# sulaimanvesal/PointCloudUDA

Hardware: AMD Instinct MI355X
Metric: adversarial train-step images/sec (seg+3 discr) at 256x256 (higher is better)
Workload: dtype bf16x3 MFMA (split-bf16, fp32 accumulate; fp32 storage); 1 GPU; MS-CMRSeg full UDA: UNet(PointNet head) + d1 + d2 + d4, 256x256x1, 4 classes; per_gpu_batch=32, global_batch=32, precision=bf16x3, parallelism=dp1, ranks_in_group=1, collective=none, streams=discriminators concurrent, d_target_forward=replayed from the adversarial pass of the same step, launch=eager (256 host cores for this rank)

## Files before the change

### pointcloududa_amd/csrc/conv_direct_d1.hip

```cpp
#include <stdlib.h>

#include "conv_host.h"
#include "conv_igemm.h"

namespace {

__device__ __forceinline__ float bf16_bits_to_float(uint16_t b) { return __builtin_bit_cast(float, (uint32_t)b << 16); }

bool direct_enabled(int bit) {
  static int mask = -1;
  if (mask < 0) {
    const char* e = getenv("PCUDA_NODIRECT");
    const char* m = getenv("PCUDA_DIRECT_MASK");
    mask = (e && atoi(e)) ? 0 : (m ? atoi(m) : 0x7f);
  }
  return (mask & bit) != 0;
}

struct D1Params {
  const float* dz; long long dz_sn, dz_sc;
  const float* x; long long x_sn, x_sc;
  float* dx; long long dx_sn, dx_sc;
  const uint16_t* wpack; int rec;
  float* partial;
  int accumulate;
  int n, h, w, oh, ow, cin, cout;
  long long cls_stride;
  int one;
};

template <int CIN>
__global__ __launch_bounds__(256) void d1_dgrad_kernel(const D1Params p) {
  __shared__ float sw[64 * CIN * 16];
  const int tid = threadIdx.x;
  for (int i = tid; i < p.cout * CIN * 16; i += 256) {
    const int kx = i & 3, ky = (i >> 2) & 3, ci = (i >> 4) % CIN, co = i / (16 * CIN);
    const int ry = ky & 1, rx = kx & 1, t = (ky >> 1) * 2 + (kx >> 1);
    const long long idx = (long long)(ry * 2 + rx) * p.cls_stride +
                          ((((long long)(co >> 5)) * 4 + t) * 32 + ci) * p.rec + (co & 31);
    const uint16_t* wq = p.wpack + idx;
    float v = bf16_bits_to_float(wq[0]);
    if (p.rec > IG_REC) v += bf16_bits_to_float(wq[32]);
    sw[i] = v;
    PCUDA_KEEP(wq);
  }
  __syncthreads();
  const int n = blockIdx.y;
  const int xg = p.w >> 3;
  const int item = blockIdx.x * 256 + tid;
  if (item >= xg * (p.h >> 1)) return;
  const int Y = item / xg, X0 = 4 * (item - Y * xg);
  float acc[CIN][2][8];
#pragma unroll
  for (int ci = 0; ci < CIN; ++ci)
#pragma unroll
    for (int r = 0; r < 2; ++r)
#pragma unroll
      for (int e = 0; e < 8; ++e) acc[ci][r][e] = 0.f;
  const float* zp = p.dz + (long long)n * p.dz_sn + (long long)Y * p.ow + X0;
  float zn[2][5];
  const float* zq[2];
#pragma unroll
  for (int a = 0; a < 2; ++a) {
    zq[a] = zp + a * p.ow;
#pragma unroll
    for (int b = 0; b < 5; ++b) zn[a][b] = zq[a][b * p.one];
  }
  for (int co = 0; co < p.cout; ++co) {
    float z[2][5];
    const float* zc[2];
#pragma unroll
    for (int a = 0; a < 2; ++a) {
      zc[a] = zq[a];
#pragma unroll
      for (int b = 0; b < 5; ++b) z[a][b] = zn[a][b];
    }
    const int con = min(co + 1, p.cout - 1);
#pragma unroll
    for (int a = 0; a < 2; ++a) {
      zq[a] = zp + (long long)con * p.dz_sc + a * p.ow;
#pragma unroll
      for (int b = 0; b < 5; ++b) zn[a][b] = zq[a][b * p.one];
    }
    const float* wc = sw + co * CIN * 16;
#pragma unroll
    for (int ci = 0; ci < CIN; ++ci)
#pragma unroll
      for (int py = 0; py < 2; ++py)
#pragma unroll
        for (int px = 0; px < 2; ++px)
#pragma unroll
          for (int a = 0; a < 2; ++a)
#pragma unroll
            for (int b = 0; b < 2; ++b) {
              const float wv = wc[(ci * 4 + py + 2 * (1 - a)) * 4 + px + 2 * (1 - b)];
#pragma unroll
              for (int j = 0; j < 4; ++j) acc[ci][py][2 * j + px] = fmaf(wv, z[a][j + b], acc[ci][py][2 * j + px]);
            }
    PCUDA_KEEP(zc[0]); PCUDA_KEEP(zc[1]);
  }
  PCUDA_KEEP(zq[0]); PCUDA_KEEP(zq[1]);
#pragma unroll
  for (int ci = 0; ci < CIN; ++ci)
#pragma unroll
    for (int r = 0; r < 2; ++r) {
      float* d = p.dx + (long long)n * p.dx_sn + (long long)ci * p.dx_sc + (long long)(2 * Y + r) * p.w + 2 * X0;
      f32x4 o0 = {acc[ci][r][0], acc[ci][r][1], acc[ci][r][2], acc[ci][r][3]};
      f32x4 o1 = {acc[ci][r][4], acc[ci][r][5], acc[ci][r][6], acc[ci][r][7]};
      if (p.accumulate) {
        const f32x4 q0 = *(const f32x4*)d, q1 = *(const f32x4*)(d + 4);
#pragma unroll
        for (int e = 0; e < 4; ++e) { o0[e] += q0[e]; o1[e] += q1[e]; }
      }
      *(f32x4*)d = o0;
      *(f32x4*)(d + 4) = o1;
    }
}

#define D1_ZP 132
#define D1_XP 276
template <int CIN>
__global__ __launch_bounds__(256) void d1_wgrad_kernel(const D1Params p, const int items) {
  extern __shared__ __attribute__((aligned(16))) float smem_f[];
  float* sz = smem_f;
  float* sx = smem_f + 64 * D1_ZP;
  const int tid = threadIdx.x;
  const int cg = tid >> 4, jg = tid & 15;
  const int ci = jg >> 2, ky = jg & 3;
  const bool live = ci < CIN;
  float acc[4][4];
#pragma unroll
  for (int c = 0; c < 4; ++c)
#pragma unroll
    for (int k = 0; k < 4; ++k) acc[c][k] = 0.f;
  const int ow4 = (p.ow + 3) >> 2;
  const int lane = tid & 63, wv = __builtin_amdgcn_readfirstlane(tid >> 6);
  float rz[16][3];
  f32x4 rx[4];
  const float* xq[4] = {p.x, p.x, p.x, p.x};
  const unsigned zoff[3] = {(unsigned)min(lane, p.ow - 1), (unsigned)min(lane + 64, p.ow - 1), (unsigned)min(lane + 128, p.ow - 1)};
  const unsigned xoff = (unsigned)min(4 * lane, p.w - 4);
  auto issue = [&](int it) {
    const int n = it / p.oh, oy = it - n * p.oh;
    const float* zb = p.dz + (long long)n * p.dz_sn + (long long)oy * p.ow;
#pragma unroll
    for (int k = 0; k < 16; ++k) {
      const float* zrow = zb + (long long)min(wv + 4 * k, p.cout - 1) * p.dz_sc;
#pragma unroll
      for (int u = 0; u < 3; ++u) rz[k][u] = zrow[zoff[u]];
    }
    const float* xb = p.x + (long long)n * p.x_sn + (long long)min(wv, CIN - 1) * p.x_sc;
#pragma unroll
    for (int r = 0; r < 4; ++r) {
      const float* xrow = xb + (long long)min(max(2 * oy + r - 2, 0), p.h - 1) * p.w;
      xq[r] = xrow + xoff;
      rx[r] = *(const f32x4*)xq[r];
    }
  };
  auto commit = [&](int it) {
    const int n = it / p.oh, oy = it - n * p.oh;
    (void)n;
#pragma unroll
    for (int k = 0; k < 16; ++k) {
      const int co = wv + 4 * k;
#pragma unroll
      for (int u = 0; u < 3; ++u) {
        const int c = lane + 64 * u;
        if (c < D1_ZP) sz[co * D1_ZP + c] = (c < p.ow && co < p.cout) ? rz[k][u] : 0.f;
      }
    }
    if (wv < CIN) {
#pragma unroll
      for (int r = 0; r < 4; ++r) {
        const int yy = 2 * oy + r - 2;
        const bool ok = (unsigned)yy < (unsigned)p.h && 4 * lane < p.w;
        float* d = sx + (wv * 4 + r) * D1_XP + 2 + 4 * lane;
#pragma unroll
        for (int e = 0; e < 4; ++e) d[e] = ok ? rx[r][e] : 0.f;
        PCUDA_KEEP(xq[r]);
        if (lane < 2) sx[(wv * 4 + r) * D1_XP + lane] = 0.f;
        if (lane < D1_XP - 2 - 256) sx[(wv * 4 + r) * D1_XP + 2 + 256 + lane] = 0.f;
      }
    }
  };
  int it = blockIdx.x;
  if (it < items) issue(it);
  for (; it < items; it += gridDim.x) {
    __syncthreads();
    commit(it);
    __syncthreads();
    const int nit = it + gridDim.x;
    if (nit < items) issue(nit);
    if (live) {
      const float* xr = sx + (ci * 4 + ky) * D1_XP;
      for (int q = 0; q < ow4; ++q) {
        const f32x4 x0 = *(const f32x4*)(xr + 8 * q), x1 = *(const f32x4*)(xr + 8 * q + 4), x2 = *(const f32x4*)(xr + 8 * q + 8);
        const float xv[12] = {x0[0], x0[1], x0[2], x0[3], x1[0], x1[1], x1[2], x1[3], x2[0], x2[1], x2[2], x2[3]};
#pragma unroll
        for (int c = 0; c < 4; ++c) {
          const f32x4 z = *(const f32x4*)(sz + (cg * 4 + c) * D1_ZP + 4 * q);
#pragma unroll
          for (int j = 0; j < 4; ++j)
#pragma unroll
            for (int kx = 0; kx < 4; ++kx) acc[c][kx] = fmaf(z[j], xv[2 * j + kx], acc[c][kx]);
        }
      }
    }
  }
  PCUDA_KEEP(zoff[0]); PCUDA_KEEP(zoff[1]); PCUDA_KEEP(zoff[2]); PCUDA_KEEP(xoff);
  if (live) {
#pragma unroll
    for (int c = 0; c < 4; ++c)
#pragma unroll
      for (int kx = 0; kx < 4; ++kx) {
        const int co = cg * 4 + c;
        if (co < p.cout) p.partial[(long long)blockIdx.x * (p.cout * CIN * 16) + ((co * CIN + ci) * 4 + ky) * 4 + kx] = acc[c][kx];
      }
  }
}

bool d1_geom(const pcuda_conv_geom* g) {
  return g->k == 4 && g->stride == 2 && g->pad == 2 && g->dil == 1 && !g->in_up && g->cin <= 5 && g->cout <= 64 &&
         (g->cout & 3) == 0 && (g->in_w & 7) == 0 && (g->in_h & 1) == 0 && g->in_w <= 256 && g->out_w <= 129;
}
const int D1_WG_BLOCKS = 768;

}

int direct_d1_dgrad(const pcuda_conv_geom* g, int prec, const pcuda_src* dy, const void* packed_w_dgrad, const pcuda_dst* dx,
                    int accumulate, size_t cls_elems, hipStream_t s, int* rc) {
  *rc = PCUDA_OK;
  if (!direct_enabled(16) || !d1_geom(g) || dy->scale1 || dy->c1 < g->cout || dx->c1 < g->cin) return 0;
  if (!aligned16(dx->p1, dx->sn1, dx->sc1)) return 0;
  D1Params p;
  memset(&p, 0, sizeof(p));
  p.dz = dy->p1; p.dz_sn = dy->sn1; p.dz_sc = dy->sc1;
  p.dx = dx->p1; p.dx_sn = dx->sn1; p.dx_sc = dx->sc1;
  p.wpack = (const uint16_t*)packed_w_dgrad; p.rec = ig_rec_bytes(prec == PCUDA_PREC_BF16X3) / 2;
  p.cls_stride = (long long)cls_elems;
  p.accumulate = accumulate;
  p.one = 1;
  p.n = g->n; p.h = g->in_h; p.w = g->in_w; p.oh = g->out_h; p.ow = g->out_w; p.cin = g->cin; p.cout = g->cout;
  const double flops = 2.0 * g->n * (double)g->out_h * g->out_w * g->cout * (double)g->cin * 16;
  char tag[96];
  snprintf(tag, sizeof(tag), "direct d1 dgrad n%d cin%d cout%d %dx%d", g->n, g->cin, g->cout, g->in_h, g->in_w);
  ProfScope prof(PCUDA_FAM_CONV_FWD, flops, s, tag);
  const dim3 grid(cdiv((long long)(g->in_w / 8) * (g->in_h / 2), 256), g->n);
  switch (g->cin) {
    case 1: hipLaunchKernelGGL(d1_dgrad_kernel<1>, grid, dim3(256), 0, s, p); break;
    case 2: hipLaunchKernelGGL(d1_dgrad_kernel<2>, grid, dim3(256), 0, s, p); break;
    case 3: hipLaunchKernelGGL(d1_dgrad_kernel<3>, grid, dim3(256), 0, s, p); break;
    case 4: hipLaunchKernelGGL(d1_dgrad_kernel<4>, grid, dim3(256), 0, s, p); break;
    default: hipLaunchKernelGGL(d1_dgrad_kernel<5>, grid, dim3(256), 0, s, p); break;
  }
  hipError_t e = hipGetLastError();
  if (e != hipSuccess) { pcuda_set_error("d1_dgrad_kernel: %s", hipGetErrorString(e)); *rc = PCUDA_E_LAUNCH; }
  return 1;
}

size_t direct_d1_wgrad_bytes(const pcuda_conv_geom* g) {
  if (!d1_geom(g) || g->cin > 4) return 0;
  return (size_t)D1_WG_BLOCKS * g->cout * g->cin * 16 * sizeof(float) + 256;
}

int direct_d1_wgrad(const WgradCall& c) {
  const pcuda_conv_geom* g = c.g;
  const pcuda_src* x = c.x;
  if (!direct_enabled(32) || !d1_geom(g) || g->cin > 4 || x->scale1 || x->c1 < g->cin || c.db) return WGRAD_NOT_TAKEN;
  if (!aligned16(x->p1, x->sn1, x->sc1)) return WGRAD_NOT_TAKEN;
  D1Params p;
  memset(&p, 0, sizeof(p));
  p.dz = c.dy; p.dz_sn = c.dy_sn; p.dz_sc = c.dy_sc;
  p.x = x->p1; p.x_sn = x->sn1; p.x_sc = x->sc1;
  p.partial = (float*)c.workspace;
  p.n = g->n; p.h = g->in_h; p.w = g->in_w; p.oh = g->out_h; p.ow = g->out_w; p.cin = g->cin; p.cout = g->cout;
  const int items = g->n * g->out_h;
  const int blocks = items < D1_WG_BLOCKS ? items : D1_WG_BLOCKS;
  const size_t lds = (size_t)(64 * D1_ZP + g->cin * 4 * D1_XP) * sizeof(float);
  const double flops = 2.0 * g->n * (double)g->out_h * g->out_w * g->cout * (double)g->cin * 16;
  char tag[96];
  snprintf(tag, sizeof(tag), "direct d1 wgrad n%d cin%d cout%d %dx%d", g->n, g->cin, g->cout, g->in_h, g->in_w);
  ProfScope prof(PCUDA_FAM_CONV_WGRAD, flops, c.s, tag);
#define D1_WG_LAUNCH(C_)                                                                                              \
  {                                                                                                                   \
              \
    if (lds > 48 * 1024) (void)hipFuncSetAttribute((const void*)d1_wgrad_kernel<C_>, hipFuncAttributeMaxDynamicSharedMemorySize, 65536); \
    hipLaunchKernelGGL(d1_wgrad_kernel<C_>, dim3(blocks), dim3(256), lds, c.s, p, items);                             \
  }
  switch (g->cin) {
    case 1: D1_WG_LAUNCH(1) break;
    case 2: D1_WG_LAUNCH(2) break;
    case 3: D1_WG_LAUNCH(3) break;
    default: D1_WG_LAUNCH(4) break;
  }
#undef D1_WG_LAUNCH
  PCUDA_CHECK_LAUNCH("d1_wgrad_kernel");
  const WgradSlabs sl = {p.partial, nullptr, (long long)g->cout * g->cin * 16, blocks, 1};
  WgradCall now = c;
  now.defer = nullptr;
  return wgrad_finish(now, sl);
}

namespace {

#define D5_MAXPIX 292
struct D5Params {
  const float* x; long long x_sn, x_sc;
  float* y; long long y_sn;
  const uint16_t* wpack; int rec;
  const float* bias;
  float slope;
  int h, w, oh, ow, cin;
};

#define D5R_NT 512
__global__ __launch_bounds__(D5R_NT) void d5_fwd_kernel(const D5Params p) {
  extern __shared__ __attribute__((aligned(16))) float d5_smem[];
  float* swt = d5_smem;
  float* spart = d5_smem + p.cin * 16;
  const int tid = threadIdx.x, n = blockIdx.x, oy = blockIdx.y;
  for (int i = tid; i < p.cin * 16; i += D5R_NT) {
    const int ci = i >> 4, t = i & 15;
    const uint16_t* wq = p.wpack + ((((long long)(ci >> 5)) * 16 + t) * 32 * p.rec + (ci & 31));
    float wv = bf16_bits_to_float(wq[0]);
    if (p.rec > IG_REC) wv += bf16_bits_to_float(wq[32]);
    PCUDA_KEEP(wq);
    swt[i] = wv;
  }
  const int ng = D5R_NT / p.ow;
  const int ox = tid % p.ow, gsel = tid / p.ow;
  const bool live = gsel < ng;
  int off[16];
#pragma unroll
  for (int t = 0; t < 16; ++t) {
    const int iy = 2 * oy + (t >> 2) - 2, ix = 2 * ox + (t & 3) - 2;
    off[t] = ((unsigned)iy < (unsigned)p.h && (unsigned)ix < (unsigned)p.w) ? iy * p.w + ix : -1;
  }
  __syncthreads();
  float acc = 0.f;
  if (live) {
    const float* xb = p.x + (long long)n * p.x_sn;
    for (int c = gsel; c < p.cin; c += ng) {
      const float* xc = xb + (long long)c * p.x_sc;
      const float* wc = swt + c * 16;
      float xv[16];
      const float* xa[16];
#pragma unroll
      for (int t = 0; t < 16; ++t) { xa[t] = xc + (off[t] >= 0 ? off[t] : 0); xv[t] = *xa[t]; }
#pragma unroll
      for (int t = 0; t < 16; ++t) acc = fmaf(wc[t], off[t] >= 0 ? xv[t] : 0.f, acc);
#pragma unroll
      for (int t = 0; t < 16; ++t) PCUDA_KEEP(xa[t]);
    }
    spart[gsel * p.ow + ox] = acc;
  }
  __syncthreads();
  if (tid < p.ow) {
    float s = 0.f;
    for (int k = 0; k < ng; ++k) s += spart[k * p.ow + tid];
    int boff = 0;
    asm volatile("" : "+v"(boff));
    s += p.bias ? p.bias[boff] : 0.f;
    PCUDA_KEEP(boff);
    s = s > 0.f ? s : s * p.slope;
    p.y[(long long)n * p.y_sn + oy * p.ow + tid] = s;
  }
}

bool d5_geom(const pcuda_conv_geom* g) {
  return g->cout == 1 && g->k == 4 && g->stride == 2 && g->pad == 2 && g->dil == 1 && !g->in_up &&
         g->in_h * g->in_w <= D5_MAXPIX && g->out_h * g->out_w <= 128;
}

}

namespace {

struct D1FParams {
  const float* x; long long x_sn, x_sc;
  float* y; long long y_sn, y_sc;
  const uint16_t* wpack; int rec;
  const float* bias; float slope;
  int n, h, w, oh, ow;
  int tiles_per_image, tiles;
};

template <bool X3, int CIN>
__global__ __launch_bounds__(256) void d1_fwd_kernel(const D1FParams p) {
  __shared__ uint4 wfrag[2][CIN * 2 * 64];
  __shared__ float sbias[64];
  const int tid = threadIdx.x, lane = tid & 63, r = lane & 31, h = lane >> 5;
  const int w = __builtin_amdgcn_readfirstlane(tid >> 6);
  {
    uint16_t* const wf = (uint16_t*)&wfrag[0][0];
    for (int e = tid; e < CIN * 2 * 64 * 8; e += 256) {
      const int j = e & 7, ln = (e >> 3) & 63, cb = (e >> 9) & 1, ks = e >> 10;
      const int tap = 8 * (ln >> 5) + j, co = cb * 32 + (ln & 31);
      const uint16_t* wq = p.wpack + ((long long)tap * 64 + co) * p.rec + ks;
      wf[e] = wq[0];
      if (X3) wf[CIN * 2 * 64 * 8 + e] = wq[32];
      PCUDA_KEEP(wq);
    }
  }
  if (tid < 64) {
    const float* bq = p.bias ? p.bias + tid : nullptr;
    sbias[tid] = bq ? *bq : 0.f;
    PCUDA_KEEP(bq);
  }
  __syncthreads();
  bf16x8 ah[CIN][2], al[CIN][2];
#pragma unroll
  for (int ks = 0; ks < CIN; ++ks)
#pragma unroll
    for (int cb = 0; cb < 2; ++cb) {
      ah[ks][cb] = __builtin_bit_cast(bf16x8, wfrag[0][(ks * 2 + cb) * 64 + lane]);
      al[ks][cb] = ah[ks][cb];
      if (X3) al[ks][cb] = __builtin_bit_cast(bf16x8, wfrag[1][(ks * 2 + cb) * 64 + lane]);
    }

  const int opix = p.oh * p.ow;
  for (int tile = blockIdx.x * 4 + w; tile < p.tiles; tile += gridDim.x * 4) {
    const int img = tile / p.tiles_per_image, pix = (tile - img * p.tiles_per_image) * 32 + r;
    const bool pv = pix < opix;
    const int pc = min(pix, opix - 1);
    const int oy = pc / p.ow, ox = pc - oy * p.ow;
    const int ix0 = 2 * ox - 2;
    const bool cv0 = (unsigned)ix0 < (unsigned)p.w, cv1 = (unsigned)(ix0 + 2) < (unsigned)p.w;
    const int cx0 = cv0 ? ix0 : 0, cx1 = cv1 ? ix0 + 2 : 0;
    int rowo[2];
    bool rv[2];
#pragma unroll
    for (int q = 0; q < 2; ++q) {
      const int iy = 2 * oy - 2 + 2 * h + q;
      rv[q] = (unsigned)iy < (unsigned)p.h;
      rowo[q] = (rv[q] ? iy : 0) * p.w;
    }
    const float* xp = p.x + (long long)img * p.x_sn;
    f32x16 acc[2];
#pragma unroll
    for (int cb = 0; cb < 2; ++cb)
#pragma unroll
      for (int i = 0; i < 16; ++i) acc[cb][i] = 0.f;
    float2 v[CIN][2][2];
    const float* pa[CIN][2][2];
#pragma unroll
    for (int ks = 0; ks < CIN; ++ks)
#pragma unroll
      for (int q = 0; q < 2; ++q) {
        const float* rp = xp + (long long)ks * p.x_sc + rowo[q];
        pa[ks][q][0] = rp + cx0;
        pa[ks][q][1] = rp + cx1;
        v[ks][q][0] = *(const float2*)pa[ks][q][0];
        v[ks][q][1] = *(const float2*)pa[ks][q][1];
      }
#pragma unroll
    for (int ks = 0; ks < CIN; ++ks) {
      float t[8];
#pragma unroll
      for (int q = 0; q < 2; ++q) {
        t[4 * q + 0] = (rv[q] & cv0) ? v[ks][q][0].x : 0.f; t[4 * q + 1] = (rv[q] & cv0) ? v[ks][q][0].y : 0.f;
        t[4 * q + 2] = (rv[q] & cv1) ? v[ks][q][1].x : 0.f; t[4 * q + 3] = (rv[q] & cv1) ? v[ks][q][1].y : 0.f;
      }
      uint4 hi, lo = make_uint4(0, 0, 0, 0);
      if (X3) {
        split2(t[0], t[1], hi.x, lo.x); split2(t[2], t[3], hi.y, lo.y);
        split2(t[4], t[5], hi.z, lo.z); split2(t[6], t[7], hi.w, lo.w);
      } else {
        hi.x = pack_bf16x2(t[0], t[1]); hi.y = pack_bf16x2(t[2], t[3]);
        hi.z = pack_bf16x2(t[4], t[5]); hi.w = pack_bf16x2(t[6], t[7]);
      }
      const bf16x8 bh = __builtin_bit_cast(bf16x8, hi), bl = __builtin_bit_cast(bf16x8, lo);
#pragma unroll
      for (int cb = 0; cb < 2; ++cb) {
        if (X3) {
          acc[cb] = __builtin_amdgcn_mfma_f32_32x32x16_bf16(al[ks][cb], bh, acc[cb], 0, 0, 0);
          acc[cb] = __builtin_amdgcn_mfma_f32_32x32x16_bf16(ah[ks][cb], bl, acc[cb], 0, 0, 0);
        }
        acc[cb] = __builtin_amdgcn_mfma_f32_32x32x16_bf16(ah[ks][cb], bh, acc[cb], 0, 0, 0);
      }
    }
#pragma unroll
    for (int ks = 0; ks < CIN; ++ks)
#pragma unroll
      for (int q = 0; q < 2; ++q) { PCUDA_KEEP(pa[ks][q][0]); PCUDA_KEEP(pa[ks][q][1]); }
    float* yp = p.y + (long long)img * p.y_sn + pc;
    if (pv) {
#pragma unroll
      for (int cb = 0; cb < 2; ++cb)
#pragma unroll
        for (int i = 0; i < 16; ++i) {
          const int co = cb * 32 + (i & 3) + 8 * (i >> 2) + 4 * h;
          float o = acc[cb][i] + sbias[co];
          o = o > 0.f ? o : o * p.slope;
          yp[(long long)co * p.y_sc] = o;
        }
    }
  }
}

}

static bool d1_fwd_on(const pcuda_conv_geom* g) {
  static int off = -1;
  if (off < 0) { const char* e = getenv("PCUDA_NO_D1FWD"); off = (e && atoi(e)) ? 1 : 0; }
  return !off && direct_enabled(16) && d1_geom(g) && g->cout == 64;
}

extern "C" int pcuda_conv2d_d1_forward_ok(const pcuda_conv_geom* g) { return (g && d1_fwd_on(g)) ? 1 : 0; }

int direct_d1_forward(const pcuda_conv_geom* g, int prec, const pcuda_src* x, const void* packed_w, const float* bias,
                      float slope, const pcuda_dst* y, float* bn_partials, hipStream_t s, int* rc) {
  *rc = PCUDA_OK;
  if (!d1_fwd_on(g) || bn_partials || x->scale1 ||
      x->c1 < g->cin || y->c1 < g->cout)
    return 0;
  if ((((uintptr_t)x->p1) & 7) || (x->sn1 & 1) || (x->sc1 & 1)) return 0;
  const bool x3 = prec == PCUDA_PREC_BF16X3;
  D1FParams p;
  memset(&p, 0, sizeof(p));
  p.x = x->p1; p.x_sn = x->sn1; p.x_sc = x->sc1;
  p.y = y->p1; p.y_sn = y->sn1; p.y_sc = y->sc1;
  p.wpack = (const uint16_t*)packed_w; p.rec = ig_rec_bytes(x3) / 2;
  p.bias = bias; p.slope = slope;
  p.n = g->n; p.h = g->in_h; p.w = g->in_w; p.oh = g->out_h; p.ow = g->out_w;
  p.tiles_per_image = (g->out_h * g->out_w + 31) / 32;
  p.tiles = p.tiles_per_image * g->n;
  const double flops = 2.0 * g->n * (double)g->out_h * g->out_w * g->cout * (double)g->cin * 16;
  char tag[96];
  snprintf(tag, sizeof(tag), "direct d1 fwd (mfma) n%d cin%d cout%d %dx%d", g->n, g->cin, g->cout, g->in_h, g->in_w);
  ProfScope prof(PCUDA_FAM_CONV_FWD, flops, s, tag);
  int grid = (p.tiles + 3) / 4;
  if (grid > 2048) grid = 2048;
#define D1F(X3_, C_) hipLaunchKernelGGL((d1_fwd_kernel<X3_, C_>), dim3(grid), dim3(256), 0, s, p)
#define D1F_C(X3_)                                                                                           \
  do {                                                                                                        \
    switch (g->cin) {                                                                                         \
      case 1: D1F(X3_, 1); break; case 2: D1F(X3_, 2); break; case 3: D1F(X3_, 3); break;                    \
      case 4: D1F(X3_, 4); break; default: D1F(X3_, 5); break;                                                \
    }                                                                                                         \
  } while (0)
  if (x3) D1F_C(true); else D1F_C(false);
#undef D1F_C
#undef D1F
  hipError_t e = hipGetLastError();
  if (e != hipSuccess) { pcuda_set_error("d1_fwd_kernel: %s", hipGetErrorString(e)); *rc = PCUDA_E_LAUNCH; }
  return 1;
}

int direct_d5_forward(const pcuda_conv_geom* g, int prec, const pcuda_src* x, const void* packed_w, const float* bias,
                      float slope, const pcuda_dst* y, float* bn_partials, hipStream_t s, int* rc) {
  *rc = PCUDA_OK;
  if (!direct_enabled(64) || !d5_geom(g) || bn_partials || x->scale1 || x->c1 < g->cin) return 0;
  D5Params p;
  p.x = x->p1; p.x_sn = x->sn1; p.x_sc = x->sc1;
  p.y = y->p1; p.y_sn = y->sn1;
  p.wpack = (const uint16_t*)packed_w; p.rec = ig_rec_bytes(prec == PCUDA_PREC_BF16X3) / 2;
  p.bias = bias; p.slope = slope;
  p.h = g->in_h; p.w = g->in_w; p.oh = g->out_h; p.ow = g->out_w; p.cin = g->cin;
  const double flops = 2.0 * g->n * (double)g->out_h * g->out_w * (double)g->cin * 16;
  char tag[96];
  snprintf(tag, sizeof(tag), "direct d5 fwd n%d cin%d %dx%d", g->n, g->cin, g->in_h, g->in_w);
  ProfScope prof(PCUDA_FAM_CONV_FWD, flops, s, tag);
  const size_t lds = (size_t)(g->cin * 16 + D5R_NT) * sizeof(float);
  if (lds > 60 * 1024) return 0;
  hipLaunchKernelGGL(d5_fwd_kernel, dim3(g->n, g->out_h), dim3(D5R_NT), lds, s, p);
  hipError_t e = hipGetLastError();
  if (e != hipSuccess) { pcuda_set_error("d5_fwd_kernel: %s", hipGetErrorString(e)); *rc = PCUDA_E_LAUNCH; }
  return 1;
}
```

Baseline: 789.2 img/s.

## Vectorize weight staging and software-pipeline input loads in direct d1/d5 conv kernels

Weight unpacking in the d1 dgrad, d1 forward and d5 forward kernels now reads packed bf16 weights as 16-byte vectors instead of scalar gathers, which adds 16-byte alignment guards on the host. The d1 dgrad inner loop double-buffers dY loads across output channels using vector loads, and the d1 forward loop prefetches the next tile's inputs before running the current tile's MFMAs. The d5 forward kernel stages input rows into LDS cooperatively, with a prefetch of the next channel pass, instead of per-thread strided gathers. The d1 forward grid cap drops from 2048 to 512 blocks, and debug-only code paths are added under a compile-time macro.

```diff
diff --git a/pointcloududa_amd/csrc/conv_direct_d1.hip b/pointcloududa_amd/csrc/conv_direct_d1.hip
--- a/pointcloududa_amd/csrc/conv_direct_d1.hip
+++ b/pointcloududa_amd/csrc/conv_direct_d1.hip
@@ -3,7 +3,13 @@
 #include "conv_host.h"
 #include "conv_igemm.h"
 
+#ifndef PCUDA_D1_DEBUG
+#define PCUDA_D1_DEBUG 0
+#endif
+
 namespace {
+
+typedef float f32x4u __attribute__((ext_vector_type(4), aligned(4)));
 
 __device__ __forceinline__ float bf16_bits_to_float(uint16_t b) { return __builtin_bit_cast(float, (uint32_t)b << 16); }
 
@@ -26,23 +32,46 @@
   int accumulate;
   int n, h, w, oh, ow, cin, cout;
   long long cls_stride;
-  int one;
 };
 
 template <int CIN>
 __global__ __launch_bounds__(256) void d1_dgrad_kernel(const D1Params p) {
   __shared__ float sw[64 * CIN * 16];
   const int tid = threadIdx.x;
-  for (int i = tid; i < p.cout * CIN * 16; i += 256) {
-    const int kx = i & 3, ky = (i >> 2) & 3, ci = (i >> 4) % CIN, co = i / (16 * CIN);
-    const int ry = ky & 1, rx = kx & 1, t = (ky >> 1) * 2 + (kx >> 1);
-    const long long idx = (long long)(ry * 2 + rx) * p.cls_stride +
-                          ((((long long)(co >> 5)) * 4 + t) * 32 + ci) * p.rec + (co & 31);
-    const uint16_t* wq = p.wpack + idx;
-    float v = bf16_bits_to_float(wq[0]);
-    if (p.rec > IG_REC) v += bf16_bits_to_float(wq[32]);
-    sw[i] = v;
-    PCUDA_KEEP(wq);
+  {
+    constexpr int ITEMS = 4 * 2 * 4 * CIN * 4, WU = (ITEMS + 255) / 256;
+    const bool x3 = p.rec > IG_REC;
+    uint4 qh[WU], ql[WU];
+    const uint16_t* wq[WU];
+    int it[WU];
+#pragma unroll
+    for (int u = 0; u < WU; ++u) {
+      int i = tid + 256 * u;
+      if (i >= ITEMS || ((i / (16 * CIN)) & 1) * 32 + 8 * (i & 3) >= p.cout) i = -1;
+      it[u] = i;
+      const int j = max(i, 0);
+      const int g8 = j & 3, ci = (j >> 2) % CIN, t = (j / (4 * CIN)) & 3, ch = (j / (16 * CIN)) & 1, cls = j / (32 * CIN);
+      wq[u] = p.wpack + ((long long)cls * p.cls_stride + (((long long)ch * 4 + t) * 32 + ci) * p.rec + 8 * g8);
+      qh[u] = *(const uint4*)wq[u];
+      ql[u] = make_uint4(0, 0, 0, 0);
+      if (x3) ql[u] = *(const uint4*)(wq[u] + 32);
+    }
+#pragma unroll
+    for (int u = 0; u < WU; ++u) {
+      const int j = max(it[u], 0);
+      const int g8 = j & 3, ci = (j >> 2) % CIN, t = (j / (4 * CIN)) & 3, ch = (j / (16 * CIN)) & 1, cls = j / (32 * CIN);
+      const int ky = (cls >> 1) + 2 * (t >> 1), kx = (cls & 1) + 2 * (t & 1);
+      const uint32_t dh[4] = {qh[u].x, qh[u].y, qh[u].z, qh[u].w}, dl[4] = {ql[u].x, ql[u].y, ql[u].z, ql[u].w};
+#pragma unroll
+      for (int k = 0; k < 8; ++k) {
+        const int co = ch * 32 + 8 * g8 + k;
+        float v = bf16_bits_to_float((uint16_t)(dh[k >> 1] >> (16 * (k & 1))));
+        if (x3) v += bf16_bits_to_float((uint16_t)(dl[k >> 1] >> (16 * (k & 1))));
+        if (it[u] >= 0 && co < p.cout) sw[((co * CIN + ci) * 4 + ky) * 4 + kx] = v;
+      }
+    }
+#pragma unroll
+    for (int u = 0; u < WU; ++u) PCUDA_KEEP(wq[u]);
   }
   __syncthreads();
   const int n = blockIdx.y;
@@ -58,30 +87,25 @@
 #pragma unroll
       for (int e = 0; e < 8; ++e) acc[ci][r][e] = 0.f;
   const float* zp = p.dz + (long long)n * p.dz_sn + (long long)Y * p.ow + X0;
-  float zn[2][5];
-  const float* zq[2];
-#pragma unroll
-  for (int a = 0; a < 2; ++a) {
-    zq[a] = zp + a * p.ow;
-#pragma unroll
-    for (int b = 0; b < 5; ++b) zn[a][b] = zq[a][b * p.one];
-  }
-  for (int co = 0; co < p.cout; ++co) {
-    float z[2][5];
-    const float* zc[2];
+  float z[2][2][5];
+  const float* zq[2][2];
+  auto request = [&](float (*zz)[5], const float** q, int co) {
+    const int con = min(co, p.cout - 1);
 #pragma unroll
     for (int a = 0; a < 2; ++a) {
-      zc[a] = zq[a];
-#pragma unroll
-      for (int b = 0; b < 5; ++b) z[a][b] = zn[a][b];
-    }
-    const int con = min(co + 1, p.cout - 1);
-#pragma unroll
-    for (int a = 0; a < 2; ++a) {
-      zq[a] = zp + (long long)con * p.dz_sc + a * p.ow;
-#pragma unroll
-      for (int b = 0; b < 5; ++b) zn[a][b] = zq[a][b * p.one];
-    }
+      q[a] = zp + (long long)con * p.dz_sc + a * p.ow;
+      if (PCUDA_D1_DEBUG == 2) {
+#pragma unroll
+        for (int b = 0; b < 5; ++b) zz[a][b] = (float)(con + b);
+      } else {
+        const f32x4u z4 = *(const f32x4u*)q[a];
+        zz[a][0] = z4[0]; zz[a][1] = z4[1]; zz[a][2] = z4[2]; zz[a][3] = z4[3];
+        zz[a][4] = q[a][4];
+      }
+    }
+    __builtin_amdgcn_sched_barrier(0);
+  };
+  auto consume = [&](const float (*zz)[5], const float** q, int co) {
     const float* wc = sw + co * CIN * 16;
 #pragma unroll
     for (int ci = 0; ci < CIN; ++ci)
@@ -95,11 +119,19 @@
             for (int b = 0; b < 2; ++b) {
               const float wv = wc[(ci * 4 + py + 2 * (1 - a)) * 4 + px + 2 * (1 - b)];
 #pragma unroll
-              for (int j = 0; j < 4; ++j) acc[ci][py][2 * j + px] = fmaf(wv, z[a][j + b], acc[ci][py][2 * j + px]);
+              for (int j = 0; j < 4; ++j) acc[ci][py][2 * j + px] = fmaf(wv, zz[a][j + b], acc[ci][py][2 * j + px]);
             }
-    PCUDA_KEEP(zc[0]); PCUDA_KEEP(zc[1]);
-  }
-  PCUDA_KEEP(zq[0]); PCUDA_KEEP(zq[1]);
+    PCUDA_KEEP(q[0]); PCUDA_KEEP(q[1]);
+  };
+  request(z[0], zq[0], 0);
+  for (int co = 0; co < p.cout; co += 2) {
+    request(z[1], zq[1], co + 1);
+    consume(z[0], zq[0], co);
+    request(z[0], zq[0], co + 2);
+    consume(z[1], zq[1], co + 1);
+  }
+  PCUDA_KEEP(zq[0][0]); PCUDA_KEEP(zq[0][1]); PCUDA_KEEP(zq[1][0]); PCUDA_KEEP(zq[1][1]);
+  if (PCUDA_D1_DEBUG == 1 && p.n >= 0) return;
 #pragma unroll
   for (int ci = 0; ci < CIN; ++ci)
 #pragma unroll
@@ -147,7 +179,7 @@
     for (int k = 0; k < 16; ++k) {
       const float* zrow = zb + (long long)min(wv + 4 * k, p.cout - 1) * p.dz_sc;
 #pragma unroll
-      for (int u = 0; u < 3; ++u) rz[k][u] = zrow[zoff[u]];
+      for (int u = 0; u < 3; ++u) rz[k][u] = PCUDA_D1_DEBUG == 2 ? (float)(k + u) : zrow[zoff[u]];
     }
     const float* xb = p.x + (long long)n * p.x_sn + (long long)min(wv, CIN - 1) * p.x_sc;
 #pragma unroll
@@ -191,7 +223,7 @@
     __syncthreads();
     const int nit = it + gridDim.x;
     if (nit < items) issue(nit);
-    if (live) {
+    if (live && !(PCUDA_D1_DEBUG == 1 && p.n >= 0)) {
       const float* xr = sx + (ci * 4 + ky) * D1_XP;
       for (int q = 0; q < ow4; ++q) {
         const f32x4 x0 = *(const f32x4*)(xr + 8 * q), x1 = *(const f32x4*)(xr + 8 * q + 4), x2 = *(const f32x4*)(xr + 8 * q + 8);
@@ -232,6 +264,7 @@
   *rc = PCUDA_OK;
   if (!direct_enabled(16) || !d1_geom(g) || dy->scale1 || dy->c1 < g->cout || dx->c1 < g->cin) return 0;
   if (!aligned16(dx->p1, dx->sn1, dx->sc1)) return 0;
+  if ((((uintptr_t)packed_w_dgrad) & 15) || (cls_elems & 7)) return 0;
   D1Params p;
   memset(&p, 0, sizeof(p));
   p.dz = dy->p1; p.dz_sn = dy->sn1; p.dz_sc = dy->sc1;
@@ -239,7 +272,6 @@
   p.wpack = (const uint16_t*)packed_w_dgrad; p.rec = ig_rec_bytes(prec == PCUDA_PREC_BF16X3) / 2;
   p.cls_stride = (long long)cls_elems;
   p.accumulate = accumulate;
-  p.one = 1;
   p.n = g->n; p.h = g->in_h; p.w = g->in_w; p.oh = g->out_h; p.ow = g->out_w; p.cin = g->cin; p.cout = g->cout;
   const double flops = 2.0 * g->n * (double)g->out_h * g->out_w * g->cout * (double)g->cin * 16;
   char tag[96];
@@ -314,18 +346,41 @@
 };
 
 #define D5R_NT 512
+#define D5_WU 2
+#define D5_XU 8
 __global__ __launch_bounds__(D5R_NT) void d5_fwd_kernel(const D5Params p) {
   extern __shared__ __attribute__((aligned(16))) float d5_smem[];
   float* swt = d5_smem;
   float* spart = d5_smem + p.cin * 16;
+  float* sx = spart + D5R_NT;
   const int tid = threadIdx.x, n = blockIdx.x, oy = blockIdx.y;
-  for (int i = tid; i < p.cin * 16; i += D5R_NT) {
-    const int ci = i >> 4, t = i & 15;
-    const uint16_t* wq = p.wpack + ((((long long)(ci >> 5)) * 16 + t) * 32 * p.rec + (ci & 31));
-    float wv = bf16_bits_to_float(wq[0]);
-    if (p.rec > IG_REC) wv += bf16_bits_to_float(wq[32]);
-    PCUDA_KEEP(wq);
-    swt[i] = wv;
+  const bool x3 = p.rec > IG_REC;
+  const int witems = ((p.cin + 31) >> 5) * 64;
+  for (int i0 = 0; i0 < witems; i0 += D5R_NT * D5_WU) {
+    uint4 qh[D5_WU], ql[D5_WU];
+    const uint16_t* wq[D5_WU];
+#pragma unroll
+    for (int u = 0; u < D5_WU; ++u) {
+      const int i = min(i0 + u * D5R_NT + tid, witems - 1);
+      wq[u] = p.wpack + ((long long)(i >> 2) * 32 * p.rec + 8 * (i & 3));
+      qh[u] = *(const uint4*)wq[u];
+      ql[u] = make_uint4(0, 0, 0, 0);
+      if (x3) ql[u] = *(const uint4*)(wq[u] + 32);
+    }
+#pragma unroll
+    for (int u = 0; u < D5_WU; ++u) {
+      const int i = i0 + u * D5R_NT + tid;
+      const int t = (i >> 2) & 15, ci0 = (i >> 6) * 32 + 8 * (i & 3);
+      const uint32_t dh[4] = {qh[u].x, qh[u].y, qh[u].z, qh[u].w}, dl[4] = {ql[u].x, ql[u].y, ql[u].z, ql[u].w};
+#pragma unroll
+      for (int k = 0; k < 8; ++k) {
+        float wv = bf16_bits_to_float((uint16_t)(dh[k >> 1] >> (16 * (k & 1))));
+        if (x3) wv += bf16_bits_to_float((uint16_t)(dl[k >> 1] >> (16 * (k & 1))));
+        if (i < witems && ci0 + k < p.cin) swt[(ci0 + k) * 16 + t] = wv;
+      }
+    }
+#pragma unroll
+    for (int u = 0; u < D5_WU; ++u) PCUDA_KEEP(wq[u]);
   }
   const int ng = D5R_NT / p.ow;
   const int ox = tid % p.ow, gsel = tid / p.ow;
@@ -334,26 +389,49 @@
 #pragma unroll
   for (int t = 0; t < 16; ++t) {
     const int iy = 2 * oy + (t >> 2) - 2, ix = 2 * ox + (t & 3) - 2;
-    off[t] = ((unsigned)iy < (unsigned)p.h && (unsigned)ix < (unsigned)p.w) ? iy * p.w + ix : -1;
-  }
-  __syncthreads();
+    off[t] = ((unsigned)iy < (unsigned)p.h && (unsigned)ix < (unsigned)p.w) ? (t >> 2) * p.w + ix : -1;
+  }
+  const int blk = 4 * p.w, pass_elems = ng * blk;
+  const float* xb = p.x + (long long)n * p.x_sn;
+  int gcl[D5_XU], goff[D5_XU];
+#pragma unroll
+  for (int u = 0; u < D5_XU; ++u) {
+    const int e = tid + D5R_NT * u, rem = e % blk, iy = 2 * oy - 2 + rem / p.w;
+    gcl[u] = e / blk;
+    goff[u] = (e < pass_elems && (unsigned)iy < (unsigned)p.h) ? (2 * oy - 2) * p.w + rem : -1;
+  }
+  float xr[D5_XU];
+  const float* xq[D5_XU];
+  auto request = [&](int k) {
+    const float* xc = xb + (long long)k * ng * p.x_sc;
+#pragma unroll
+    for (int u = 0; u < D5_XU; ++u) {
+      const bool ok = goff[u] >= 0 && k * ng + gcl[u] < p.cin;
+      xq[u] = ok ? xc + ((long long)gcl[u] * p.x_sc + goff[u]) : xb;
+      xr[u] = *xq[u];
+    }
+  };
+  const int npass = (p.cin + ng - 1) / ng;
   float acc = 0.f;
-  if (live) {
-    const float* xb = p.x + (long long)n * p.x_sn;
-    for (int c = gsel; c < p.cin; c += ng) {
-      const float* xc = xb + (long long)c * p.x_sc;
+  request(0);
+  for (int k = 0; k < npass; ++k) {
+    __syncthreads();
+#pragma unroll
+    for (int u = 0; u < D5_XU; ++u)
+      if (tid + D5R_NT * u < pass_elems) sx[tid + D5R_NT * u] = xr[u];
+#pragma unroll
+    for (int u = 0; u < D5_XU; ++u) PCUDA_KEEP(xq[u]);
+    __syncthreads();
+    if (k + 1 < npass) request(k + 1);
+    const int c = k * ng + gsel;
+    if (live && c < p.cin) {
       const float* wc = swt + c * 16;
-      float xv[16];
-      const float* xa[16];
-#pragma unroll
-      for (int t = 0; t < 16; ++t) { xa[t] = xc + (off[t] >= 0 ? off[t] : 0); xv[t] = *xa[t]; }
-#pragma unroll
-      for (int t = 0; t < 16; ++t) acc = fmaf(wc[t], off[t] >= 0 ? xv[t] : 0.f, acc);
-#pragma unroll
-      for (int t = 0; t < 16; ++t) PCUDA_KEEP(xa[t]);
-    }
-    spart[gsel * p.ow + ox] = acc;
-  }
+      const float* xs = sx + gsel * blk;
+#pragma unroll
+      for (int t = 0; t < 16; ++t) acc = fmaf(wc[t], off[t] >= 0 ? xs[max(off[t], 0)] : 0.f, acc);
+    }
+  }
+  if (live) spart[gsel * p.ow + ox] = acc;
   __syncthreads();
   if (tid < p.ow) {
     float s = 0.f;
@@ -385,6 +463,10 @@
   int tiles_per_image, tiles;
 };
 
+#ifndef D1_FWD_BLOCKS
+#define D1_FWD_BLOCKS 512
+#endif
+
 template <bool X3, int CIN>
 __global__ __launch_bounds__(256) void d1_fwd_kernel(const D1FParams p) {
   __shared__ uint4 wfrag[2][CIN * 2 * 64];
@@ -393,14 +475,28 @@
   const int w = __builtin_amdgcn_readfirstlane(tid >> 6);
   {
     uint16_t* const wf = (uint16_t*)&wfrag[0][0];
-    for (int e = tid; e < CIN * 2 * 64 * 8; e += 256) {
-      const int j = e & 7, ln = (e >> 3) & 63, cb = (e >> 9) & 1, ks = e >> 10;
-      const int tap = 8 * (ln >> 5) + j, co = cb * 32 + (ln & 31);
-      const uint16_t* wq = p.wpack + ((long long)tap * 64 + co) * p.rec + ks;
-      wf[e] = wq[0];
-      if (X3) wf[CIN * 2 * 64 * 8 + e] = wq[32];
-      PCUDA_KEEP(wq);
-    }
+    uint4 qh[4], ql[4];
+    const uint16_t* wq[4];
+#pragma unroll
+    for (int u = 0; u < 4; ++u) {
+      wq[u] = p.wpack + (long long)(tid + 256 * u) * p.rec;
+      qh[u] = *(const uint4*)wq[u];
+      ql[u] = qh[u];
+      if (X3) ql[u] = *(const uint4*)(wq[u] + 32);
+    }
+#pragma unroll
+    for (int u = 0; u < 4; ++u) {
+      const int tap = (tid + 256 * u) >> 6, co = tid & 63;
+      const int e0 = ((co >> 5) * 64 + (tap >> 3) * 32 + (co & 31)) * 8 + (tap & 7);
+      const uint32_t dh[4] = {qh[u].x, qh[u].y, qh[u].z, qh[u].w}, dl[4] = {ql[u].x, ql[u].y, ql[u].z, ql[u].w};
+#pragma unroll
+      for (int ks = 0; ks < CIN; ++ks) {
+        wf[e0 + ks * 1024] = (uint16_t)(dh[ks >> 1] >> (16 * (ks & 1)));
+        if (X3) wf[CIN * 2 * 64 * 8 + e0 + ks * 1024] = (uint16_t)(dl[ks >> 1] >> (16 * (ks & 1)));
+      }
+    }
+#pragma unroll
+    for (int u = 0; u < 4; ++u) PCUDA_KEEP(wq[u]);
   }
   if (tid < 64) {
     const float* bq = p.bias ? p.bias + tid : nullptr;
@@ -419,30 +515,27 @@
     }
 
   const int opix = p.oh * p.ow;
-  for (int tile = blockIdx.x * 4 + w; tile < p.tiles; tile += gridDim.x * 4) {
-    const int img = tile / p.tiles_per_image, pix = (tile - img * p.tiles_per_image) * 32 + r;
-    const bool pv = pix < opix;
-    const int pc = min(pix, opix - 1);
-    const int oy = pc / p.ow, ox = pc - oy * p.ow;
+  struct Tile { int img, pc; bool pv, cv0, cv1, rv[2]; };
+  Tile nx = {0, 0, false, false, false, {false, false}};
+  float2 v[CIN][2][2];
+  const float* pa[CIN][2][2];
+  auto request = [&](int tile) {
+    nx.img = tile / p.tiles_per_image;
+    const int pix = (tile - nx.img * p.tiles_per_image) * 32 + r;
+    nx.pv = pix < opix;
+    nx.pc = min(pix, opix - 1);
+    const int oy = nx.pc / p.ow, ox = nx.pc - oy * p.ow;
     const int ix0 = 2 * ox - 2;
-    const bool cv0 = (unsigned)ix0 < (unsigned)p.w, cv1 = (unsigned)(ix0 + 2) < (unsigned)p.w;
-    const int cx0 = cv0 ? ix0 : 0, cx1 = cv1 ? ix0 + 2 : 0;
+    nx.cv0 = (unsigned)ix0 < (unsigned)p.w; nx.cv1 = (unsigned)(ix0 + 2) < (unsigned)p.w;
+    const int cx0 = nx.cv0 ? ix0 : 0, cx1 = nx.cv1 ? ix0 + 2 : 0;
     int rowo[2];
-    bool rv[2];
 #pragma unroll
     for (int q = 0; q < 2; ++q) {
       const int iy = 2 * oy - 2 + 2 * h + q;
-      rv[q] = (unsigned)iy < (unsigned)p.h;
-      rowo[q] = (rv[q] ? iy : 0) * p.w;
-    }
-    const float* xp = p.x + (long long)img * p.x_sn;
-    f32x16 acc[2];
-#pragma unroll
-    for (int cb = 0; cb < 2; ++cb)
-#pragma unroll
-      for (int i = 0; i < 16; ++i) acc[cb][i] = 0.f;
-    float2 v[CIN][2][2];
-    const float* pa[CIN][2][2];
+      nx.rv[q] = (unsigned)iy < (unsigned)p.h;
+      rowo[q] = (nx.rv[q] ? iy : 0) * p.w;
+    }
+    const float* xp = p.x + (long long)nx.img * p.x_sn;
 #pragma unroll
     for (int ks = 0; ks < CIN; ++ks)
 #pragma unroll
@@ -450,16 +543,25 @@
         const float* rp = xp + (long long)ks * p.x_sc + rowo[q];
         pa[ks][q][0] = rp + cx0;
         pa[ks][q][1] = rp + cx1;
-        v[ks][q][0] = *(const float2*)pa[ks][q][0];
-        v[ks][q][1] = *(const float2*)pa[ks][q][1];
-      }
+        v[ks][q][0] = PCUDA_D1_DEBUG == 2 ? make_float2((float)lane, (float)ks) : *(const float2*)pa[ks][q][0];
+        v[ks][q][1] = PCUDA_D1_DEBUG == 2 ? make_float2((float)q, (float)lane) : *(const float2*)pa[ks][q][1];
+      }
+  };
+  const int tstep = gridDim.x * 4;
+  int tile = blockIdx.x * 4 + w;
+  if (tile < p.tiles) request(tile);
+  for (; tile < p.tiles; tile += tstep) {
+    const Tile cu = nx;
+    const int img = cu.img, pc = cu.pc;
+    const bool pv = cu.pv;
+    bf16x8 bh[CIN], bl[CIN];
 #pragma unroll
     for (int ks = 0; ks < CIN; ++ks) {
       float t[8];
 #pragma unroll
       for (int q = 0; q < 2; ++q) {
-        t[4 * q + 0] = (rv[q] & cv0) ? v[ks][q][0].x : 0.f; t[4 * q + 1] = (rv[q] & cv0) ? v[ks][q][0].y : 0.f;
-        t[4 * q + 2] = (rv[q] & cv1) ? v[ks][q][1].x : 0.f; t[4 * q + 3] = (rv[q] & cv1) ? v[ks][q][1].y : 0.f;
+        t[4 * q + 0] = (cu.rv[q] & cu.cv0) ? v[ks][q][0].x : 0.f; t[4 * q + 1] = (cu.rv[q] & cu.cv0) ? v[ks][q][0].y : 0.f;
+        t[4 * q + 2] = (cu.rv[q] & cu.cv1) ? v[ks][q][1].x : 0.f; t[4 * q + 3] = (cu.rv[q] & cu.cv1) ? v[ks][q][1].y : 0.f;
       }
       uint4 hi, lo = make_uint4(0, 0, 0, 0);
       if (X3) {
@@ -469,22 +571,31 @@
         hi.x = pack_bf16x2(t[0], t[1]); hi.y = pack_bf16x2(t[2], t[3]);
         hi.z = pack_bf16x2(t[4], t[5]); hi.w = pack_bf16x2(t[6], t[7]);
       }
-      const bf16x8 bh = __builtin_bit_cast(bf16x8, hi), bl = __builtin_bit_cast(bf16x8, lo);
+      bh[ks] = __builtin_bit_cast(bf16x8, hi);
+      bl[ks] = __builtin_bit_cast(bf16x8, lo);
+    }
+#pragma unroll
+    for (int ks = 0; ks < CIN; ++ks)
+#pragma unroll
+      for (int q = 0; q < 2; ++q) { PCUDA_KEEP(pa[ks][q][0]); PCUDA_KEEP(pa[ks][q][1]); }
+    if (tile + tstep < p.tiles) request(tile + tstep);
+    f32x16 acc[2];
+#pragma unroll
+    for (int cb = 0; cb < 2; ++cb)
+#pragma unroll
+      for (int i = 0; i < 16; ++i) acc[cb][i] = 0.f;
+#pragma unroll
+    for (int ks = 0; ks < CIN; ++ks)
 #pragma unroll
       for (int cb = 0; cb < 2; ++cb) {
         if (X3) {
-          acc[cb] = __builtin_amdgcn_mfma_f32_32x32x16_bf16(al[ks][cb], bh, acc[cb], 0, 0, 0);
-          acc[cb] = __builtin_amdgcn_mfma_f32_32x32x16_bf16(ah[ks][cb], bl, acc[cb], 0, 0, 0);
+          acc[cb] = __builtin_amdgcn_mfma_f32_32x32x16_bf16(al[ks][cb], bh[ks], acc[cb], 0, 0, 0);
+          acc[cb] = __builtin_amdgcn_mfma_f32_32x32x16_bf16(ah[ks][cb], bl[ks], acc[cb], 0, 0, 0);
         }
-        acc[cb] = __builtin_amdgcn_mfma_f32_32x32x16_bf16(ah[ks][cb], bh, acc[cb], 0, 0, 0);
-      }
-    }
-#pragma unroll
-    for (int ks = 0; ks < CIN; ++ks)
-#pragma unroll
-      for (int q = 0; q < 2; ++q) { PCUDA_KEEP(pa[ks][q][0]); PCUDA_KEEP(pa[ks][q][1]); }
-    float* yp = p.y + (long long)img * p.y_sn + pc;
-    if (pv) {
+        acc[cb] = __builtin_amdgcn_mfma_f32_32x32x16_bf16(ah[ks][cb], bh[ks], acc[cb], 0, 0, 0);
+      }
+    float* yq = p.y + (long long)img * p.y_sn + pc + (long long)(4 * h) * p.y_sc;
+    if (pv && !(PCUDA_D1_DEBUG == 1 && p.n >= 0)) {
 #pragma unroll
       for (int cb = 0; cb < 2; ++cb)
 #pragma unroll
@@ -492,7 +603,8 @@
           const int co = cb * 32 + (i & 3) + 8 * (i >> 2) + 4 * h;
           float o = acc[cb][i] + sbias[co];
           o = o > 0.f ? o : o * p.slope;
-          yp[(long long)co * p.y_sc] = o;
+          *yq = o;
+          yq += ((i & 3) == 3 ? 5 : 1) * p.y_sc;
         }
     }
   }
@@ -515,6 +627,7 @@
       x->c1 < g->cin || y->c1 < g->cout)
     return 0;
   if ((((uintptr_t)x->p1) & 7) || (x->sn1 & 1) || (x->sc1 & 1)) return 0;
+  if (((uintptr_t)packed_w) & 15) return 0;
   const bool x3 = prec == PCUDA_PREC_BF16X3;
   D1FParams p;
   memset(&p, 0, sizeof(p));
@@ -530,7 +643,7 @@
   snprintf(tag, sizeof(tag), "direct d1 fwd (mfma) n%d cin%d cout%d %dx%d", g->n, g->cin, g->cout, g->in_h, g->in_w);
   ProfScope prof(PCUDA_FAM_CONV_FWD, flops, s, tag);
   int grid = (p.tiles + 3) / 4;
-  if (grid > 2048) grid = 2048;
+  if (grid > D1_FWD_BLOCKS) grid = D1_FWD_BLOCKS;
 #define D1F(X3_, C_) hipLaunchKernelGGL((d1_fwd_kernel<X3_, C_>), dim3(grid), dim3(256), 0, s, p)
 #define D1F_C(X3_)                                                                                           \
   do {                                                                                                        \
@@ -551,6 +664,7 @@
                       float slope, const pcuda_dst* y, float* bn_partials, hipStream_t s, int* rc) {
   *rc = PCUDA_OK;
   if (!direct_enabled(64) || !d5_geom(g) || bn_partials || x->scale1 || x->c1 < g->cin) return 0;
+  if (((uintptr_t)packed_w) & 15) return 0;
   D5Params p;
   p.x = x->p1; p.x_sn = x->sn1; p.x_sc = x->sc1;
   p.y = y->p1; p.y_sn = y->sn1;
@@ -561,8 +675,9 @@
   char tag[96];
   snprintf(tag, sizeof(tag), "direct d5 fwd n%d cin%d %dx%d", g->n, g->cin, g->in_h, g->in_w);
   ProfScope prof(PCUDA_FAM_CONV_FWD, flops, s, tag);
-  const size_t lds = (size_t)(g->cin * 16 + D5R_NT) * sizeof(float);
-  if (lds > 60 * 1024) return 0;
+  if ((size_t)(g->cin * 16 + D5R_NT) * sizeof(float) > 60 * 1024) return 0;
+  const size_t lds = (size_t)(g->cin * 16 + D5R_NT + (D5R_NT / g->out_w) * 4 * g->in_w) * sizeof(float);
+  if (lds > 48 * 1024) (void)hipFuncSetAttribute((const void*)d5_fwd_kernel, hipFuncAttributeMaxDynamicSharedMemorySize, 80 * 1024);
   hipLaunchKernelGGL(d5_fwd_kernel, dim3(g->n, g->out_h), dim3(D5R_NT), lds, s, p);
   hipError_t e = hipGetLastError();
   if (e != hipSuccess) { pcuda_set_error("d5_fwd_kernel: %s", hipGetErrorString(e)); *rc = PCUDA_E_LAUNCH; }
```

After: 792.7 img/s, median of 6. Within noise of the previous version (+0.4%).
